# JiawangBian/SC-SfMLearner-Release

Hardware: AMD Instinct MI355X
Metric: train images/sec (+ warp-loss ms/step) KITTI 256x832 RN18 (higher is better)
Workload: dtype f32; 1 GPU; configs[1]: kitti 256x832, batch 12/GPU, 2 refs (seq 3), ResNet18 DispNet + ResNet18 PoseNet, ssim+mask+auto-mask, zeros padding, 1 scale; global_batch=12, parallelism=1 GPU, memory_format=contiguous (NCHW)

## Files before the change

__graft_entry__.py:

```python
import os
import sys

ROOT = os.path.dirname(os.path.abspath(__file__))
PKG = os.path.join(ROOT, "sc-sfmlearner-release_amd")
for p in (ROOT, PKG):
    if p not in sys.path:
        sys.path.insert(0, p)


def build() -> None:
    from scsfm_hip import _lib, build as hip_build
    path = hip_build.build(force=False)
    lib = _lib.CLib(path)
    assert lib._dll.scsfm_abi_version() == _lib.ABI_VERSION
    nets_path = hip_build.build_nets(force=False)
    nets = _lib.CLib(nets_path, _lib.NETS_HEADER, _lib.NETS_ABI_VERSION, "scsfm_nets_")
    eval_path = hip_build.build_eval(force=False)
    ev = _lib.CLib(eval_path, _lib.EVAL_HEADER, _lib.EVAL_ABI_VERSION, "scsfm_eval_")
    odom_path = hip_build.build_odom(force=False)
    od = _lib.CLib(odom_path, _lib.ODOM_HEADER, _lib.ODOM_ABI_VERSION, "scsfm_odom_")
    enc_path = hip_build.build_enc(force=False)
    enc = _lib.CLib(enc_path, _lib.ENC_HEADER, _lib.ENC_ABI_VERSION, "scsfm_enc_")
    stem_path = hip_build.build_stem(force=False)
    stem = _lib.CLib(stem_path, _lib.STEM_HEADER, _lib.STEM_ABI_VERSION, "scsfm_stem_")
    snip_path = hip_build.build_snip(force=False)
    snip = _lib.CLib(snip_path, _lib.SNIP_HEADER, _lib.SNIP_ABI_VERSION, "scsfm_snip_")
    prep_path = hip_build.build_prep(force=False)
    prep = _lib.CLib(prep_path, _lib.PREP_HEADER, _lib.PREP_ABI_VERSION, "scsfm_prep_")
    vis_path = hip_build.build_vis(force=False)
    vis = _lib.CLib(vis_path, _lib.VIS_HEADER, _lib.VIS_ABI_VERSION, "scsfm_vis_")
    dvis_path = hip_build.build_dvis(force=False)
    dvis = _lib.CLib(dvis_path, _lib.DVIS_HEADER, _lib.DVIS_ABI_VERSION, "scsfm_dvis_")
    val_path = hip_build.build_val(force=False)
    val = _lib.CLib(val_path, _lib.VAL_HEADER, _lib.VAL_ABI_VERSION, "scsfm_val_")
    enceval_path = hip_build.build_enceval(force=False)
    enceval = _lib.CLib(enceval_path, _lib.ENCEVAL_HEADER, _lib.ENCEVAL_ABI_VERSION, "scsfm_enceval_")
    decb_path = hip_build.build_decb(force=False)
    decb = _lib.CLib(decb_path, _lib.DECB_HEADER, _lib.DECB_ABI_VERSION, "scsfm_decb_")
    wrw_path = hip_build.build_wrw(force=False)
    wrw = _lib.CLib(wrw_path, _lib.WRW_HEADER, _lib.WRW_ABI_VERSION, "scsfm_wrw_")
    vlog_path = hip_build.build_vlog(force=False)
    vlog = _lib.CLib(vlog_path, _lib.VLOG_HEADER, _lib.VLOG_ABI_VERSION, "scsfm_vlog_")
    import inverse_warp
    import loss_functions
    import models
    from scsfm_hip import decoder, depth_eval, depth_vis, encoder, odometry, prepare, snippets, visualise
    from scsfm_hip import conv_wrw, decoder_bias, encoder_eval, validation, validation_log
    from oracle import scsfm_oracle
    print(f"[vlog:build] {vlog_path}: {len(vlog.decls)} entry points resolved")
    print(f"[wrw:build] {wrw_path}: {len(wrw.decls)} entry points resolved")
    print(f"[decb:build] {decb_path}: {len(decb.decls)} entry points resolved")
    print(f"[enceval:build] {enceval_path}: {len(enceval.decls)} entry points resolved")
    print(f"[val:build] {val_path}: {len(val.decls)} entry points resolved")
    print(f"[build:dvis] {dvis_path}: {len(dvis.decls)} entry points resolved")
    print(f"[build] {path}: {len(lib.decls)} entry points resolved")
    print(f"[build] {nets_path}: {len(nets.decls)} entry points resolved")
    print(f"[build] {eval_path}: {len(ev.decls)} entry points resolved")
    print(f"[build] {odom_path}: {len(od.decls)} entry points resolved")
    print(f"[build] {enc_path}: {len(enc.decls)} entry points resolved")
    print(f"[build] {stem_path}: {len(stem.decls)} entry points resolved")
    print(f"[build] {snip_path}: {len(snip.decls)} entry points resolved")
    print(f"[build:vis] {vis_path}: {len(vis.decls)} entry points resolved")
    print(f"[build:prep] {prep_path}: {len(prep.decls)} entry points resolved")


def smoke() -> None:
    import torch

    import loss_functions as LF
    from oracle import scsfm_oracle as O
    from scsfm_hip import _lib, synth

    assert torch.cuda.is_available(), "smoke() needs a HIP device"
    lib = _lib.get()
    assert lib.path.endswith("libscsfm_hip.so")
    dev = torch.device("cuda:0")
    d = synth.make_batch(2, 128, 416, n_ref=2, seed=0, depth="smooth")

    def leaves(device):
        mv = lambda t: t.to(device).clone().requires_grad_(True)
        return ([mv(t) for t in d["tgt_depth"]], [[mv(t) for t in r] for r in d["ref_depths"]],
# ... 86 lines not shown
    assert _lib.get_enceval().path.endswith("libscsfm_enceval.so")
    bn_e = nn.BatchNorm2d(4).to(dev)
    with torch.no_grad():
        bn_e.running_mean.copy_(torch.tensor([0.5, -1.0, 0.0, 2.0]))
        bn_e.running_var.copy_(torch.tensor([0.25, 1.0, 4.0, 0.5]))
        bn_e.weight.copy_(torch.tensor([1.0, -0.5, 2.0, 0.0]))
        bn_e.bias.copy_(torch.tensor([0.0, 0.1, -0.2, 0.3]))
    bn_e.eval()
    with torch.no_grad():
        f0_e, pooled_e = EE.bn_act(xs, bn_e, pool=True)
        want_e = F.relu(bn_e(xs))
        assert torch.equal(f0_e, EE.bn_act(xs, bn_e)) and torch.equal(pooled_e, F.max_pool2d(f0_e, 3, 2, 1))
        assert torch.equal(pooled_e, EE.max_pool(f0_e))
    err_e = float((f0_e - want_e).abs().max())
    print(f"[smoke] enceval: eval-mode BatchNorm / ReLU / max-pool, max |fused - ATen| {err_e:.2e}")
    assert err_e <= 1e-5
    from scsfm_hip import decoder_bias as DB
    assert _lib.get_decb().path.endswith("libscsfm_decb.so")
    conv_b = nn.Conv2d(4, 3, 3).to(dev)
    xb = torch.randn(2, 4, 9, 11, device=dev)
    want_b = F.pad(F.elu(conv_b(xb)), (1, 1, 1, 1), mode="reflect")
    want_h = 10 * torch.sigmoid(conv_b(xb)) + 0.01
    (want_b.sum() + want_h.sum()).backward()
    want_gb = conv_b.bias.grad.clone()
    conv_b.bias.grad = None
    raw = F.conv2d(xb, conv_b.weight, None)
    got_b, got_h = DB.elu_pad(raw, conv_b.bias), DB.disp_head(raw, conv_b.bias, 10, 0.01)
    (got_b.sum() + got_h.sum()).backward()
    err_b = float((conv_b.bias.grad - want_gb).abs().max() / want_gb.abs().max())
    print(f"[smoke] decb: bias folded into elu_pad and disp_head, relative bias-gradient difference {err_b:.2e}")
    assert torch.equal(got_b, want_b) and float((got_h - want_h).abs().max()) <= 1e-6 and err_b <= 1e-5
    _smoke_wrw(dev)
    _smoke_vlog(dev)
    print("[smoke] ok")


def _smoke_wrw(dev) -> None:
    import torch
    import torch.nn.functional as F

    from scsfm_hip import _lib
    from scsfm_hip import conv_wrw as CW
    assert _lib.get_wrw().path.endswith("libscsfm_wrw.so")
    xw = torch.randn(2, 16, 7, 69, device=dev, requires_grad=True)
    ww = torch.randn(16, 16, 3, 3, device=dev, requires_grad=True)
    gy = torch.randn(2, 16, 5, 67, device=dev)
    gx_w, gw_w = torch.autograd.grad(CW.conv3x3_valid(xw, ww), (xw, ww), gy)
    gx_m, gw_m = torch.autograd.grad(F.conv2d(xw, ww), (xw, ww), gy)
    gw_64 = torch.autograd.grad(F.conv2d(xw.double(), ww.double()), ww, gy.double())[0]
    s_64 = torch.autograd.grad(F.conv2d(xw.double().abs(), ww.double()), ww, gy.double().abs())[0]
    err_w, err_m = float((gw_w - gw_64).abs().max()), float((gw_m - gw_64).abs().max())
    print(f"[smoke] wrw: weight gradient of a 16 -> 16 convolution, max |hip - fp64| {err_w:.2e} (MIOpen's {err_m:.2e})")
    assert float((gx_w - gx_m).abs().max()) <= 1e-5 * float(gx_m.abs().max())
    assert err_w <= 2 * err_m + 8 * 2.0 ** -24 * float(s_64.max())
    assert torch.equal(gw_w, CW.weight_grad(xw.detach(), gy))


def _smoke_vlog(dev) -> None:
    import numpy as np
    import torch

    from scsfm_hip import _lib
    from scsfm_hip import validation_log as VL
    assert _lib.get_vlog().path.endswith("libscsfm_vlog.so")
    ramp = torch.linspace(0.05, 12.0, 35).reshape(1, 5, 7)
    r = ramp.numpy()
    for cmap, max_value in (("magma", None), ("rainbow", 10)):
        floats, rgba = VL.map_pictures(ramp.to(dev), cmap, max_value)
        table = VL.colour_table_f32(cmap)
        d = r.max() if max_value is None else np.float32(max_value)
        xa = (r / d).astype(np.float32) * np.float32(len(table))
        want = table[np.clip(xa.astype(np.int64), 0, len(table) - 1)]
        assert floats.shape == (1, 4, 5, 7) and np.array_equal(floats.cpu().numpy(), want.transpose(0, 3, 1, 2)), cmap
        assert rgba.shape == (1, 5, 7, 4) and np.array_equal(rgba.cpu().numpy(), VL.to_bytes(want)), cmap
        assert torch.equal(VL.tensor2array(ramp[0].to(dev), max_value, cmap), floats[0])
    print("[smoke] vlog: magma and rainbow pictures of a ramp equal the table lookup, as floats and as bytes")


if __name__ == "__main__":
    build()
    if "--smoke" in sys.argv:
        smoke()
```

sc-sfmlearner-release_amd/models/DispResNet.py:

```python
from __future__ import absolute_import, division, print_function

import numpy as np
import torch
import torch.nn as nn
import torch.nn.functional as F

from .resnet_encoder import ResnetEncoder


class Conv3x3(nn.Module):
    def __init__(self, in_channels, out_channels, use_refl=True):
        super().__init__()
        self.pad = nn.ReflectionPad2d(1) if use_refl else nn.ZeroPad2d(1)
        self.conv = nn.Conv2d(int(in_channels), int(out_channels), 3)

    def forward(self, x):
        return self.conv(self.pad(x))


class ConvBlock(nn.Module):
    def __init__(self, in_channels, out_channels):
        super().__init__()
        self.conv = Conv3x3(in_channels, out_channels)
        self.nonlin = nn.ELU(inplace=True)
# ... 54 lines not shown
            x = self.decoder[self._up[(i, 0)]](x)
            x = F.interpolate(x, scale_factor=2, mode="nearest")
            if self.use_skips and i > 0:
                x = torch.cat([x, feats[i - 1]], 1)
            x = self.decoder[self._up[(i, 1)]](x)
            if i in self._head:
                outputs.append(self.alpha * self.sigmoid(self.decoder[self._head[i]](x)) + self.beta)
        return outputs[::-1]

    def forward_fused(self, feats):
        from scsfm_hip import conv_wrw as CW, decoder as D

        def conv(k, x):
            m = self._conv(k)
            if CW.applies(x, m):
                y = CW.conv3x3_valid(x, m.weight)
                return y if m.bias is None else y + m.bias.view(1, -1, 1, 1)
            return m(x)

        outputs = []
        x = D.pad(feats[-1])
        for i in range(4, -1, -1):
            a = conv(self._up[(i, 0)], x)
            x = D.up_cat_pad(a, feats[i - 1] if self.use_skips and i > 0 else None)
            b = conv(self._up[(i, 1)], x)
            if i == 0 and i not in self._head:
                break
            x = D.elu_pad(b)
            if i in self._head:
                outputs.append(self.alpha * self.sigmoid(conv(self._head[i], x)) + self.beta)
        return outputs[::-1]

    def forward_fused_bias(self, feats):
        from scsfm_hip import conv_wrw as CW, decoder as D, decoder_bias as DB

        def conv(k, x):
            m = self._conv(k)
            if CW.applies(x, m):
                return CW.conv3x3_valid(x, m.weight), m.bias
            return F.conv2d(x, m.weight, None, m.stride, m.padding, m.dilation, m.groups), m.bias

        outputs = []
        x = D.pad(feats[-1])
        for i in range(4, -1, -1):
            a, bias = conv(self._up[(i, 0)], x)
            x = DB.up_cat_pad(a, bias, feats[i - 1] if self.use_skips and i > 0 else None)
            if i == 0 and i not in self._head:
                self._conv(self._up[(i, 1)])(x)
                break
            b, bias = conv(self._up[(i, 1)], x)
            x = DB.elu_pad(b, bias)
            if i in self._head:
                h, bias = conv(self._head[i], x)
                outputs.append(DB.disp_head(h, bias, self.alpha, self.beta))
        return outputs[::-1]


class DispResNet(nn.Module):
    def __init__(self, num_layers=18, pretrained=True):
        super().__init__()
        self.encoder = ResnetEncoder(num_layers=num_layers, pretrained=pretrained, num_input_images=1)
        self.decoder = DepthDecoder(self.encoder.num_ch_enc)

    def init_weights(self):
        pass

    def forward(self, x):
        outputs = self.decoder(self.encoder(x))
        return outputs if self.training else outputs[0]
```

sc-sfmlearner-release_amd/scsfm_hip/_lib.py:

```python
from __future__ import annotations

import ctypes
import os
import re
import threading

import torch

HERE = os.path.dirname(os.path.abspath(__file__))
HEADER = os.path.join(os.path.dirname(os.path.dirname(HERE)), "include", "scsfm_hip.h")
LIB_PATH = os.environ.get("SCSFM_HIP_LIB") or os.path.join(HERE, "libscsfm_hip.so")

ABI_VERSION = 9

_CTYPES = {"int": ctypes.c_int, "unsigned": ctypes.c_uint, "size_t": ctypes.c_size_t, "double": ctypes.c_double,
           "float": ctypes.c_float}
_DECL = re.compile(r"^(int|size_t)\s+(scsfm_\w+)\s*\(([^)]*)\)\s*;", re.M | re.S)


def parse_header(path=HEADER):
    text = open(path).read()
    text = re.sub(r"/\*.*?\*/", "", text, flags=re.S)
    out = {}
    for ret, name, args in _DECL.findall(text):
# ... 420 lines not shown
                lib = CLib(WRW_LIB_PATH, WRW_HEADER, WRW_ABI_VERSION, "scsfm_wrw_")
                if lib.source_id() != _build.wrw_source_id():
                    raise ScsfmError(f"{WRW_LIB_PATH}: its source id {lib.source_id()} is not the tree's "
                                     f"{_build.wrw_source_id()}")
                _wrw = lib
    return _wrw


VLOG_HEADER = os.path.join(os.path.dirname(os.path.dirname(HERE)), "include", "scsfm_vlog.h")
VLOG_LIB_PATH = os.path.join(HERE, "libscsfm_vlog.so")
VLOG_ABI_VERSION = 1
_vlog = None


def get_vlog() -> CLib:
    global _vlog
    if _vlog is None:
        with _lock:
            if _vlog is None:
                from . import build as _build
                if _build.vlog_is_stale():
                    have = _build.binary_source_id(VLOG_LIB_PATH)
                    try:
                        _build.build_vlog()
                    except Exception as e:
                        raise ScsfmError(f"{VLOG_LIB_PATH} is stale or missing ({have}) and cannot be built here: {e}") \
                            from e
                lib = CLib(VLOG_LIB_PATH, VLOG_HEADER, VLOG_ABI_VERSION, "scsfm_vlog_")
                if lib.source_id() != _build.vlog_source_id():
                    raise ScsfmError(f"{VLOG_LIB_PATH}: its source id {lib.source_id()} is not the tree's "
                                     f"{_build.vlog_source_id()}")
                _vlog = lib
    return _vlog
```

sc-sfmlearner-release_amd/scsfm_hip/build.py:

```python
from __future__ import annotations

import contextlib
import fcntl
import glob
import hashlib
import os
import shutil
import subprocess
import sys
import tempfile

HERE = os.path.dirname(os.path.abspath(__file__))
CSRC = os.path.join(os.path.dirname(HERE), "csrc")
LIB = os.path.join(HERE, "libscsfm_hip.so")
LOCK = LIB + ".lock"
LOG = LIB + ".buildlog"
INCLUDE = os.path.join(os.path.dirname(os.path.dirname(HERE)), "include")
NETS_CSRC = os.path.join(os.path.dirname(HERE), "csrc_nets")
NETS_LIB = os.path.join(HERE, "libscsfm_nets.so")
EVAL_CSRC = os.path.join(os.path.dirname(HERE), "csrc_eval")
EVAL_LIB = os.path.join(HERE, "libscsfm_eval.so")
ODOM_CSRC = os.path.join(os.path.dirname(HERE), "csrc_odom")
ODOM_LIB = os.path.join(HERE, "libscsfm_odom.so")
ENC_CSRC = os.path.join(os.path.dirname(HERE), "csrc_enc")
ENC_LIB = os.path.join(HERE, "libscsfm_enc.so")
STEM_CSRC = os.path.join(os.path.dirname(HERE), "csrc_stem")
STEM_LIB = os.path.join(HERE, "libscsfm_stem.so")
SNIP_CSRC = os.path.join(os.path.dirname(HERE), "csrc_snip")
SNIP_LIB = os.path.join(HERE, "libscsfm_snip.so")
PREP_CSRC = os.path.join(os.path.dirname(HERE), "csrc_prep")
PREP_LIB = os.path.join(HERE, "libscsfm_prep.so")
VIS_CSRC = os.path.join(os.path.dirname(HERE), "csrc_vis")
VIS_LIB = os.path.join(HERE, "libscsfm_vis.so")
DVIS_CSRC = os.path.join(os.path.dirname(HERE), "csrc_dvis")
DVIS_LIB = os.path.join(HERE, "libscsfm_dvis.so")
VAL_CSRC = os.path.join(os.path.dirname(HERE), "csrc_val")
VAL_LIB = os.path.join(HERE, "libscsfm_val.so")
ENCEVAL_CSRC = os.path.join(os.path.dirname(HERE), "csrc_enceval")
ENCEVAL_LIB = os.path.join(HERE, "libscsfm_enceval.so")
DECB_CSRC = os.path.join(os.path.dirname(HERE), "csrc_decb")
DECB_LIB = os.path.join(HERE, "libscsfm_decb.so")
WRW_CSRC = os.path.join(os.path.dirname(HERE), "csrc_wrw")
WRW_LIB = os.path.join(HERE, "libscsfm_wrw.so")
VLOG_CSRC = os.path.join(os.path.dirname(HERE), "csrc_vlog")
VLOG_LIB = os.path.join(HERE, "libscsfm_vlog.so")
ARCH = "gfx950"
FLAGS = ["-O3", "-std=c++17", "-fPIC", "-shared", f"--offload-arch={ARCH}", "-munsafe-fp-atomics",
         "-fno-gpu-rdc", "-Wall", "-Wno-unused-function",
         "-fno-slp-vectorize"]
ID_MARKER = b"scsfm-source-id:"


def sources():
    return sorted(glob.glob(os.path.join(CSRC, "*.hip")))


def deps():
    return sources() + sorted(glob.glob(os.path.join(CSRC, "*.h"))) + \
        [os.path.join(INCLUDE, "scsfm_hip.h")]


def nets_sources():
    return sorted(glob.glob(os.path.join(NETS_CSRC, "*.hip")))


def nets_deps():
    return nets_sources() + sorted(glob.glob(os.path.join(NETS_CSRC, "*.h"))) + [os.path.join(INCLUDE, "scsfm_nets.h")]


def eval_sources():
    return sorted(glob.glob(os.path.join(EVAL_CSRC, "*.hip")))


def eval_deps():
    return eval_sources() + sorted(glob.glob(os.path.join(EVAL_CSRC, "*.h"))) + [os.path.join(INCLUDE, "scsfm_eval.h")]


def odom_sources():
# ... 61 lines not shown


def enceval_sources():
    return sorted(glob.glob(os.path.join(ENCEVAL_CSRC, "*.hip")))


def enceval_deps():
    return enceval_sources() + sorted(glob.glob(os.path.join(ENCEVAL_CSRC, "*.h"))) + \
        [os.path.join(INCLUDE, "scsfm_enceval.h")]


def decb_sources():
    return sorted(glob.glob(os.path.join(DECB_CSRC, "*.hip")))


def decb_deps():
    return decb_sources() + sorted(glob.glob(os.path.join(DECB_CSRC, "*.h"))) + [os.path.join(INCLUDE, "scsfm_decb.h")]


def wrw_sources():
    return sorted(glob.glob(os.path.join(WRW_CSRC, "*.hip")))


def wrw_deps():
    return wrw_sources() + sorted(glob.glob(os.path.join(WRW_CSRC, "*.h"))) + [os.path.join(INCLUDE, "scsfm_wrw.h")]


def vlog_sources():
    return sorted(glob.glob(os.path.join(VLOG_CSRC, "*.hip")))


def vlog_deps():
    return vlog_sources() + sorted(glob.glob(os.path.join(VLOG_CSRC, "*.h"))) + [os.path.join(INCLUDE, "scsfm_vlog.h")]


def _hash(files, extra=()):
    h = hashlib.sha256()
    for path in files:
        h.update(os.path.basename(path).encode())
        h.update(open(path, "rb").read())
    h.update(" ".join(FLAGS).encode())
    if extra:
        h.update(b"\0extra:" + " ".join(extra).encode())
    return h.hexdigest()[:16]


def source_id(extra=()):
    files = deps()
    if any("SCSFM_WITH_MARCH" in e or "variants" in e for e in extra):
        vsrc = os.path.join(os.path.dirname(os.path.dirname(HERE)), "variants", "src")
        files = files + sorted(p for p in glob.glob(os.path.join(vsrc, "*")) if os.path.isfile(p))
    return _hash(files, extra)


def nets_source_id():
    return _hash(nets_deps())


def eval_source_id():
    return _hash(eval_deps())


def odom_source_id():
    return _hash(odom_deps())


# ... 9 lines not shown
    return _hash(snip_deps())


def prep_source_id():
    return _hash(prep_deps())


def vis_source_id():
    return _hash(vis_deps())


def dvis_source_id():
    return _hash(dvis_deps())


def val_source_id():
    return _hash(val_deps())


def enceval_source_id():
    return _hash(enceval_deps())


def decb_source_id():
    return _hash(decb_deps())


def wrw_source_id():
    return _hash(wrw_deps())


def vlog_source_id():
    return _hash(vlog_deps())


def binary_source_id(path=LIB):
    try:
        blob = open(path, "rb").read()
    except OSError:
        return None
    i = blob.find(ID_MARKER)
    if i < 0:
        return None
    j = i + len(ID_MARKER)
    return blob[j:j + 16].decode("ascii", "replace")


def is_stale():
    return binary_source_id(LIB) != source_id()


def nets_is_stale():
    return binary_source_id(NETS_LIB) != nets_source_id()


def eval_is_stale():
    return binary_source_id(EVAL_LIB) != eval_source_id()


def odom_is_stale():
    return binary_source_id(ODOM_LIB) != odom_source_id()


def enc_is_stale():
    return binary_source_id(ENC_LIB) != enc_source_id()

# ... 6 lines not shown
    return binary_source_id(SNIP_LIB) != snip_source_id()


def prep_is_stale():
    return binary_source_id(PREP_LIB) != prep_source_id()


def vis_is_stale():
    return binary_source_id(VIS_LIB) != vis_source_id()


def dvis_is_stale():
    return binary_source_id(DVIS_LIB) != dvis_source_id()


def val_is_stale():
    return binary_source_id(VAL_LIB) != val_source_id()


def enceval_is_stale():
    return binary_source_id(ENCEVAL_LIB) != enceval_source_id()


def decb_is_stale():
    return binary_source_id(DECB_LIB) != decb_source_id()


def wrw_is_stale():
    return binary_source_id(WRW_LIB) != wrw_source_id()


def vlog_is_stale():
    return binary_source_id(VLOG_LIB) != vlog_source_id()


@contextlib.contextmanager
def _build_lock(lock=None):
    fd = os.open(lock or LOCK, os.O_CREAT | os.O_RDWR, 0o644)
    try:
        fcntl.flock(fd, fcntl.LOCK_EX)
        yield
    finally:
        try:
            fcntl.flock(fd, fcntl.LOCK_UN)
        finally:
            os.close(fd)


def build(force=False, verbose=True, extra=()):
    extra = tuple(extra)
    return _build(LIB, source_id(extra), sources(), extra, force, verbose)


def build_nets(force=False, verbose=True):
    return _build(NETS_LIB, nets_source_id(), nets_sources(), ("-I", INCLUDE), force, verbose)


def build_eval(force=False, verbose=True):
    return _build(EVAL_LIB, eval_source_id(), eval_sources(), ("-I", INCLUDE), force, verbose)


def build_odom(force=False, verbose=True):
    return _build(ODOM_LIB, odom_source_id(), odom_sources(), ("-I", INCLUDE), force, verbose)


def build_enc(force=False, verbose=True):
# ... 8 lines not shown
    return _build(SNIP_LIB, snip_source_id(), snip_sources(), ("-I", INCLUDE), force, verbose)


def build_prep(force=False, verbose=True):
    return _build(PREP_LIB, prep_source_id(), prep_sources(), ("-I", INCLUDE), force, verbose)


def build_vis(force=False, verbose=True):
    return _build(VIS_LIB, vis_source_id(), vis_sources(), ("-I", INCLUDE), force, verbose)


def build_dvis(force=False, verbose=True):
    return _build(DVIS_LIB, dvis_source_id(), dvis_sources(), ("-I", INCLUDE), force, verbose)


def build_val(force=False, verbose=True):
    return _build(VAL_LIB, val_source_id(), val_sources(), ("-I", INCLUDE), force, verbose)


def build_enceval(force=False, verbose=True):
    return _build(ENCEVAL_LIB, enceval_source_id(), enceval_sources(), ("-I", INCLUDE), force, verbose)


def build_decb(force=False, verbose=True):
    return _build(DECB_LIB, decb_source_id(), decb_sources(), ("-I", INCLUDE), force, verbose)


def build_wrw(force=False, verbose=True):
    return _build(WRW_LIB, wrw_source_id(), wrw_sources(), ("-I", INCLUDE), force, verbose)


def build_vlog(force=False, verbose=True):
    return _build(VLOG_LIB, vlog_source_id(), vlog_sources(), ("-I", INCLUDE), force, verbose)


def _build(lib, want, srcs, extra, force, verbose):
    if not force and binary_source_id(lib) == want:
        return lib
    with _build_lock(lib + ".lock"):
        if not force and binary_source_id(lib) == want:
            return lib
        hipcc = shutil.which("hipcc") or "/opt/rocm/bin/hipcc"
        name = os.path.basename(lib)
        if not os.path.exists(hipcc):
            raise RuntimeError(f"hipcc not found: {name} cannot be built on this machine")
        fd, tmp = tempfile.mkstemp(prefix=name[:-len(".so")] + ".", suffix=f".{os.getpid()}.tmp", dir=HERE)
        os.close(fd)
        try:
            cmd = [hipcc, *FLAGS, f'-DSCSFM_SOURCE_ID="{want}"', *extra, "-o", tmp, *srcs]
            if verbose:
                print("[scsfm_hip.build]", " ".join(cmd), flush=True)
            subprocess.run(cmd, check=True)
            os.chmod(tmp, 0o755)
            os.replace(tmp, lib)
            with open(lib + ".buildlog", "a") as f:
                f.write(f"{want} {os.getpid()}\n")
        finally:
            if os.path.exists(tmp):
                os.unlink(tmp)
    return lib


if __name__ == "__main__":
    build(force="--force" in sys.argv)
    build_nets(force="--force" in sys.argv)
    build_eval(force="--force" in sys.argv)
    build_odom(force="--force" in sys.argv)
    build_enc(force="--force" in sys.argv)
    build_stem(force="--force" in sys.argv)
    build_snip(force="--force" in sys.argv)
    build_prep(force="--force" in sys.argv)
    build_vis(force="--force" in sys.argv)
    build_dvis(force="--force" in sys.argv)
    build_val(force="--force" in sys.argv)
    build_enceval(force="--force" in sys.argv)
    build_decb(force="--force" in sys.argv)
    build_wrw(force="--force" in sys.argv)
    build_vlog(force="--force" in sys.argv)
    print(LIB)
    print(NETS_LIB)
    print(EVAL_LIB)
    print(ODOM_LIB)
    print(ENC_LIB)
    print(STEM_LIB)
    print(SNIP_LIB)
    print(PREP_LIB)
    print(VIS_LIB)
    print(DVIS_LIB)
    print(VAL_LIB)
    print(ENCEVAL_LIB)
    print(DECB_LIB)
    print(WRW_LIB)
    print(VLOG_LIB)
```

sc-sfmlearner-release_amd/scsfm_hip/config.py:

```python
from __future__ import annotations

_hint = (1.0, 0.5)
_hint_dev = {}


def set_weight_hint(w_photo, w_geom):
    global _hint
    if w_photo is None:
        _hint = None
        return
    import numpy as np
    _hint = (float(np.float32(w_photo)), float(np.float32(w_geom)))
    for t in _hint_dev.values():
        t.copy_(t.new_tensor(_hint))


def weight_hint():
    return _hint


def hint_tensor(device):
    if _hint is None:
        return None
    import torch
# ... 42 lines not shown
    _errors_torch = bool(on)


_decoder_bias = None


def decoder_bias_folded():
    global _decoder_bias
    if _decoder_bias is None:
        import os
        _decoder_bias = os.environ.get("SCSFM_DECODER_BIAS", "1") != "0"
    return _decoder_bias


def set_decoder_bias_folded(on):
    global _decoder_bias
    _decoder_bias = None if on is None else bool(on)


_decoder_wrw = None


def decoder_wrw():
    global _decoder_wrw
    if _decoder_wrw is None:
        import os
        _decoder_wrw = os.environ.get("SCSFM_DECODER_WRW", "1") != "0"
    return _decoder_wrw


def set_decoder_wrw(on):
    global _decoder_wrw
    _decoder_wrw = None if on is None else bool(on)
```

sc-sfmlearner-release_amd/scsfm_hip/conv_wrw.py:

```python
from __future__ import annotations

import torch
import torch.nn.functional as F

from . import _lib, config
from .capi import _stream

COUT = (1, 16, 32)
CIN = (16, 32, 64, 96)
ROUTED = {(64, 32), (96, 32), (32, 16), (16, 16), (64, 1), (32, 1), (16, 1)}


def covers(cin, cout):
    return int(cin) in CIN and int(cout) in COUT


def applies(x, m):
    w = m.weight
    return (config.decoder_wrw() and x.is_cuda and x.dtype == torch.float32 and x.dim() == 4 and x.is_contiguous()
            and w.is_cuda and w.dtype == torch.float32 and w.is_contiguous() and tuple(w.shape[2:]) == (3, 3)
            and tuple(m.stride) == (1, 1) and tuple(m.padding) == (0, 0) and tuple(m.dilation) == (1, 1)
            and m.groups == 1 and m.padding_mode == "zeros" and x.shape[1] == w.shape[1]
            and (int(w.shape[1]), int(w.shape[0])) in ROUTED and x.shape[2] >= 3 and x.shape[3] >= 3)


def weight_grad(x, gy):
    B, Cin, Hp, Wp = x.shape
    Cout, H, W = gy.shape[1], Hp - 2, Wp - 2
    if not (x.is_cuda and gy.is_cuda and x.dtype == gy.dtype == torch.float32 and x.is_contiguous()
            and gy.is_contiguous() and tuple(gy.shape) == (B, Cout, H, W)):
        raise ValueError(f"scsfm_hip.conv_wrw: CUDA fp32 contiguous x[B, Cin, H + 2, W + 2] and gy[B, Cout, H, W] only "
                         f"(got {x.device} {x.dtype} {tuple(x.shape)} and {gy.device} {gy.dtype} {tuple(gy.shape)})")
    lib = _lib.get_wrw()
    n = lib.size("scsfm_wrw_conv3x3_ws_bytes", B, Cin, Cout, H, W)
    if n == 0:
        raise ValueError(f"scsfm_hip.conv_wrw: no kernel for {Cin} -> {Cout} channels at {B} x {H} x {W}")
    ws = torch.empty(n // 4, dtype=torch.float32, device=x.device)
    dw = torch.empty((Cout, Cin, 3, 3), dtype=torch.float32, device=x.device)
    lib.call("scsfm_wrw_conv3x3_f32", B, Cin, Cout, H, W, x.data_ptr(), gy.data_ptr(), dw.data_ptr(), ws.data_ptr(), n,
             _stream(x))
    return dw


class _Conv3x3Valid(torch.autograd.Function):
    @staticmethod
    def forward(ctx, x, weight):
        ctx.save_for_backward(x, weight)
        return F.conv2d(x, weight)

    @staticmethod
    def backward(ctx, gy):
        x, weight = ctx.saved_tensors
        gy = gy.contiguous()
        gx = gw = None
        if ctx.needs_input_grad[0]:
            gx = torch.ops.aten.convolution_backward(gy, x, weight, None, [1, 1], [0, 0], [1, 1], False, [0, 0], 1,
                                                     [True, False, False])[0]
        if ctx.needs_input_grad[1]:
            gw = weight_grad(x, gy)
        return gx, gw


def conv3x3_valid(x_padded, weight):
    return _Conv3x3Valid.apply(x_padded, weight)
```

Baseline: 149.4 images/s.

## Fuse disparity head tail backward and add MFMA conv3x3 data-gradient kernel

Adds a HIP library with two kernels. The first runs the whole backward of the final decoder stage (sigmoid-scaled disparity head, its 16->1 conv data gradient with reflect-pad folding, and ELU backward) in one kernel, with fp64 bias-gradient sums. The second is an MFMA-based 16/32<-16 channel 3x3 conv data-gradient kernel that replaces MIOpen's backward-data call for routed decoder convs. Both aim to cut kernel launches, intermediate memory traffic and MIOpen overhead in the decoder backward pass, at the cost of more custom code and border-handling complexity.

```diff
diff --git a/__graft_entry__.py b/__graft_entry__.py
--- a/__graft_entry__.py
+++ b/__graft_entry__.py
@@ -41,12 +41,15 @@
     wrw = _lib.CLib(wrw_path, _lib.WRW_HEADER, _lib.WRW_ABI_VERSION, "scsfm_wrw_")
     vlog_path = hip_build.build_vlog(force=False)
     vlog = _lib.CLib(vlog_path, _lib.VLOG_HEADER, _lib.VLOG_ABI_VERSION, "scsfm_vlog_")
+    dgrad_path = hip_build.build_dgrad(force=False)
+    dgrad = _lib.CLib(dgrad_path, _lib.DGRAD_HEADER, _lib.DGRAD_ABI_VERSION, "scsfm_dgrad_")
     import inverse_warp
     import loss_functions
     import models
     from scsfm_hip import decoder, depth_eval, depth_vis, encoder, odometry, prepare, snippets, visualise
-    from scsfm_hip import conv_wrw, decoder_bias, encoder_eval, validation, validation_log
+    from scsfm_hip import conv_wrw, decoder_bias, decoder_dgrad, encoder_eval, validation, validation_log
     from oracle import scsfm_oracle
+    print(f"[dgrad:build] {dgrad_path}: {len(dgrad.decls)} entry points resolved")
     print(f"[vlog:build] {vlog_path}: {len(vlog.decls)} entry points resolved")
     print(f"[wrw:build] {wrw_path}: {len(wrw.decls)} entry points resolved")
     print(f"[decb:build] {decb_path}: {len(decb.decls)} entry points resolved")
@@ -199,6 +202,7 @@
     assert torch.equal(got_b, want_b) and float((got_h - want_h).abs().max()) <= 1e-6 and err_b <= 1e-5
     _smoke_wrw(dev)
     _smoke_vlog(dev)
+    _smoke_dgrad(dev)
     print("[smoke] ok")
 
 
@@ -244,6 +248,42 @@
     print("[smoke] vlog: magma and rainbow pictures of a ramp equal the table lookup, as floats and as bytes")
 
 
+def _smoke_dgrad(dev) -> None:
+    import torch
+    import torch.nn.functional as F
+
+    from scsfm_hip import _lib
+    from scsfm_hip import decoder_bias as DB, decoder_dgrad as DG
+    assert _lib.get_dgrad().path.endswith("libscsfm_dgrad.so")
+    g = torch.Generator().manual_seed(3)
+    b, bias = torch.randn(2, 16, 5, 67, generator=g), torch.randn(16, generator=g)
+    wh, bh = torch.randn(1, 16, 3, 3, generator=g) / 12, torch.randn(1, generator=g)
+    gy = torch.randn(2, 1, 5, 67, generator=g)
+    leaves = lambda dtype: [t.to(dev, dtype).requires_grad_(True) for t in (b, bias, wh, bh)]
+
+    def chain(b, bias, wh, bh):
+        q = F.pad(F.elu(b + bias.view(1, -1, 1, 1)), (1, 1, 1, 1), mode="reflect")
+        return 10 * torch.sigmoid(F.conv2d(q, wh, bh)) + 0.01
+    x32, x64 = leaves(torch.float32), leaves(torch.float64)
+    out = DG.head_tail(*x32, 10, 0.01)
+    got = torch.autograd.grad(out, x32, gy.to(dev))
+    want = torch.autograd.grad(chain(*x64), x64, gy.to(dev).double())
+    with torch.no_grad():
+        parts = DB.disp_head(F.conv2d(DB.elu_pad(x32[0], x32[1]), x32[2]), x32[3], 10, 0.01)
+    assert torch.equal(out, parts)
+    err = max(float((a.double() - c).abs().max() / c.abs().max()) for a, c in zip(got, want))
+    print(f"[smoke] dgrad: the tail's backward in one kernel, largest relative gradient difference to fp64 {err:.2e}")
+    assert err <= 1e-5
+    from scsfm_hip import conv_wrw as CW
+    gyc, wc = torch.randn(2, 16, 5, 67, generator=g).to(dev), torch.randn(16, 16, 3, 3, generator=g).to(dev)
+    xc = torch.zeros(2, 16, 7, 69, device=dev)
+    want_c = torch.ops.aten.convolution_backward(gyc, xc, wc, None, [1, 1], [0, 0], [1, 1], False, [0, 0], 1,
+                                                 [True, False, False])[0]
+    err_c = float((CW.data_grad(gyc, wc) - want_c).abs().max() / want_c.abs().max())
+    print(f"[smoke] dgrad: data gradient of a 16 -> 16 convolution, relative difference to MIOpen's {err_c:.2e}")
+    assert err_c <= 1e-5
+
+
 if __name__ == "__main__":
     build()
     if "--smoke" in sys.argv:
diff --git a/include/scsfm_dgrad.h b/include/scsfm_dgrad.h
--- /dev/null
+++ b/include/scsfm_dgrad.h
@@ -0,0 +1,30 @@
+#ifndef SCSFM_DGRAD_H_
+#define SCSFM_DGRAD_H_
+
+#include <stddef.h>
+
+#ifndef SCSFM_ERR_ARG
+#define SCSFM_ERR_ARG (-1)
+#endif
+
+#ifdef __cplusplus
+extern "C" {
+#endif
+
+int scsfm_dgrad_abi_version(void);
+int scsfm_dgrad_source_id(char* buf, size_t n);
+int scsfm_dgrad_head_tail_covers(int C);
+size_t scsfm_dgrad_head_tail_ws_bytes(int B, int C, int H, int W);
+int scsfm_dgrad_head_tail_bwd_f32(int B, int C, int H, int W, float alpha, const float* q, const float* y,
+                                  const float* g_out, const float* w, float* g, float* g_b, void* ws, size_t ws_bytes,
+                                  float* g_bias_b, float* g_bias_head, void* stream);
+
+int scsfm_dgrad_conv3x3_covers(int Cin, int Cout);
+int scsfm_dgrad_conv3x3_f32(int B, int Cin, int Cout, int H, int W, const float* dy, const float* w, float* dx,
+                            void* stream);
+
+#ifdef __cplusplus
+}
+#endif
+
+#endif
diff --git a/sc-sfmlearner-release_amd/csrc_dgrad/scsfm_conv_dgrad.hip b/sc-sfmlearner-release_amd/csrc_dgrad/scsfm_conv_dgrad.hip
--- /dev/null
+++ b/sc-sfmlearner-release_amd/csrc_dgrad/scsfm_conv_dgrad.hip
@@ -0,0 +1,125 @@
+#include <hip/hip_runtime.h>
+
+#include "scsfm_dgrad.h"
+
+#ifndef SCSFM_WRW_F32X4
+typedef float f32x4 __attribute__((ext_vector_type(4)));
+#endif
+
+namespace scsfm_dgrad_conv {
+
+constexpr int kCout = 16;
+constexpr int kWave = 64;
+constexpr int kWaves = 4;
+constexpr int kThreads = kWave * kWaves;
+constexpr int kTP = 8, kTQ = 64;
+constexpr int kLH = kTP + 2, kLW = kTQ + 2;
+constexpr int kPlane = 672;
+constexpr int kSteps = 36;
+constexpr int kBatch = 14;
+
+template <int NB>
+__global__ __launch_bounds__(kThreads) void conv3x3_dgrad_kernel(int H, int W, int tiles_q, int tiles_p,
+                                                                  const float* __restrict__ dy,
+                                                                  const float* __restrict__ w, float* __restrict__ dx) {
+  __shared__ float tile[kCout * kPlane];
+  constexpr int Cin = 16 * NB;
+  const int tid = threadIdx.x, lane = tid & (kWave - 1), wv = tid >> 6;
+  const int col = lane & 15, quad = lane >> 4;
+  int t = blockIdx.x;
+  const int tq = t % tiles_q;
+  t /= tiles_q;
+  const int tp = t % tiles_p, n = t / tiles_p;
+  const int p0 = tp * kTP, q0 = tq * kTQ;
+  const int Hp = H + 2, Wp = W + 2;
+
+  float a[NB][kSteps];
+#pragma unroll
+  for (int m = 0; m < NB; ++m)
+#pragma unroll
+    for (int rs = 0; rs < 9; ++rs)
+#pragma unroll
+      for (int g = 0; g < 4; ++g) a[m][rs * 4 + g] = w[((4 * g + quad) * Cin + 16 * m + col) * 9 + rs];
+
+  constexpr int kElems = kCout * kLH * kLW;
+  for (int e0 = tid; e0 < kElems; e0 += kBatch * kThreads) {
+    float v[kBatch];
+    int at[kBatch];
+#pragma unroll
+    for (int u = 0; u < kBatch; ++u) {
+      const int e = e0 + u * kThreads;
+      const int co = e / (kLH * kLW), rem = e - co * (kLH * kLW);
+      const int lr = rem / kLW, lc = rem - lr * kLW;
+      const int gi = p0 - 2 + lr, gj = q0 - 2 + lc;
+      at[u] = e < kElems ? co * kPlane + rem : -1;
+      v[u] = 0.f;
+      if (e < kElems && gi >= 0 && gi < H && gj >= 0 && gj < W) v[u] = dy[((n * kCout + co) * H + gi) * W + gj];
+    }
+#pragma unroll
+    for (int u = 0; u < kBatch; ++u)
+      if (at[u] >= 0) tile[at[u]] = v[u];
+  }
+  __syncthreads();
+
+#pragma unroll 1
+  for (int k = 0; k < kTP / kWaves; ++k) {
+    const int lp = wv + k * kWaves, p = p0 + lp;
+#pragma unroll 1
+    for (int cb = 0; cb < kTQ / 16; ++cb) {
+      f32x4 acc[NB];
+#pragma unroll
+      for (int m = 0; m < NB; ++m) acc[m] = f32x4{0.f, 0.f, 0.f, 0.f};
+      const float* base = tile + quad * kPlane + (lp + 2) * kLW + cb * 16 + col + 2;
+#pragma unroll
+      for (int r = 0; r < 3; ++r)
+#pragma unroll
+        for (int s = 0; s < 3; ++s)
+#pragma unroll
+          for (int g = 0; g < 4; ++g) {
+            const float b = base[4 * g * kPlane - r * kLW - s];
+#pragma unroll
+            for (int m = 0; m < NB; ++m)
+              acc[m] = __builtin_amdgcn_mfma_f32_16x16x4f32(a[m][(r * 3 + s) * 4 + g], b, acc[m], 0, 0, 0);
+          }
+      const int q = q0 + cb * 16 + col;
+      if (p < Hp && q < Wp) {
+#pragma unroll
+        for (int m = 0; m < NB; ++m)
+#pragma unroll
+          for (int i = 0; i < 4; ++i) dx[((n * Cin + 16 * m + 4 * quad + i) * Hp + p) * Wp + q] = acc[m][i];
+      }
+    }
+  }
+}
+
+inline int ceil_div(int a, int b) { return (a + b - 1) / b; }
+
+inline long long workgroups(int B, int Cin, int Cout, int H, int W) {
+  if (B <= 0 || Cout != kCout || (Cin != 16 && Cin != 32) || H < 1 || W < 1) return 0;
+  if ((long long)B * (Cin > Cout ? Cin : Cout) * (H + 2ll) * (W + 2ll) >= (1ll << 31)) return 0;
+  return (long long)B * ceil_div(H + 2, kTP) * ceil_div(W + 2, kTQ);
+}
+
+}
+
+using namespace scsfm_dgrad_conv;
+
+extern "C" {
+
+int scsfm_dgrad_conv3x3_covers(int Cin, int Cout) { return Cout == kCout && (Cin == 16 || Cin == 32) ? 1 : 0; }
+
+int scsfm_dgrad_conv3x3_f32(int B, int Cin, int Cout, int H, int W, const float* dy, const float* w, float* dx,
+                            void* stream) {
+  const long long nwg = workgroups(B, Cin, Cout, H, W);
+  if (nwg == 0 || !dy || !w || !dx) return SCSFM_ERR_ARG;
+  (void)hipGetLastError();
+  const int tiles_q = ceil_div(W + 2, kTQ), tiles_p = ceil_div(H + 2, kTP);
+  const dim3 grid((unsigned)nwg), block(kThreads);
+  if (Cin == 16)
+    hipLaunchKernelGGL(conv3x3_dgrad_kernel<1>, grid, block, 0, (hipStream_t)stream, H, W, tiles_q, tiles_p, dy, w, dx);
+  else
+    hipLaunchKernelGGL(conv3x3_dgrad_kernel<2>, grid, block, 0, (hipStream_t)stream, H, W, tiles_q, tiles_p, dy, w, dx);
+  return (int)hipGetLastError();
+}
+
+}
diff --git a/sc-sfmlearner-release_amd/csrc_dgrad/scsfm_decoder_dgrad.hip b/sc-sfmlearner-release_amd/csrc_dgrad/scsfm_decoder_dgrad.hip
--- /dev/null
+++ b/sc-sfmlearner-release_amd/csrc_dgrad/scsfm_decoder_dgrad.hip
@@ -0,0 +1,218 @@
+#include <hip/hip_runtime.h>
+
+#include <stdint.h>
+
+#include "scsfm_dgrad.h"
+
+#pragma clang fp contract(off)
+
+namespace scsfm_dgrad {
+
+constexpr int kC = 16;
+constexpr int kWave = 64;
+constexpr int kWaves = 4;
+constexpr int kThreads = kWave * kWaves;
+constexpr int kTW = 64, kTH = 8;
+constexpr int kLW = kTW + 2, kLH = kTH + 2;
+constexpr int kSums = kC + 1;
+
+__device__ inline float elu_grad(float g, float r) { return r <= 0.f ? g * (r + 1.f) : g; }
+
+__device__ inline double wave_sum(double v) {
+#pragma unroll
+  for (int d = kWave / 2; d > 0; d >>= 1) v += __shfl_down(v, d);
+  return v;
+}
+
+template <bool SUM>
+__global__ __launch_bounds__(kThreads) void head_tail_bwd_kernel(int H, int W, int tiles_x, int tiles_y, float alpha,
+                                                                  const float* __restrict__ q,
+                                                                  const float* __restrict__ y,
+                                                                  const float* __restrict__ g_out,
+                                                                  const float* __restrict__ w, float* __restrict__ g,
+                                                                  float* __restrict__ g_b, double* __restrict__ ws) {
+  __shared__ float tile[kLH * kLW];
+  __shared__ double red[kWaves][kSums];
+  const int tid = threadIdx.x, lane = tid & (kWave - 1), wv = tid >> 6;
+  int t = blockIdx.x;
+  const int tx = t % tiles_x;
+  t /= tiles_x;
+  const int ty = t % tiles_y, b = t / tiles_y;
+  const int i0 = ty * kTH, j0 = tx * kTW;
+
+  for (int e = tid; e < kLH * kLW; e += kThreads) {
+    const int li = e / kLW, lj = e - li * kLW;
+    const int gi = i0 + li - 1, gj = j0 + lj - 1;
+    float v = 0.f;
+    if (gi >= 0 && gi < H && gj >= 0 && gj < W) {
+      const int idx = (b * H + gi) * W + gj;
+      v = g_out[idx];
+      if (y) {
+        const float s = y[idx];
+        v = ((v * alpha) * (1.f - s)) * s;
+      }
+      if (li >= 1 && li <= kTH && lj >= 1 && lj <= kTW) g[idx] = v;
+    }
+    tile[e] = v;
+  }
+  __syncthreads();
+
+  const int Hp = H + 2, Wp = W + 2;
+  const int j = j0 + lane;
+  double sum[kSums];
+#pragma unroll
+  for (int c = 0; c < kSums; ++c) sum[c] = 0.0;
+
+  auto gat = [&](int gi, int gj) -> float {
+    return gi >= 0 && gi < H && gj >= 0 && gj < W ? tile[(gi - i0 + 1) * kLW + (gj - j0 + 1)] : 0.f;
+  };
+  auto gq = [&](const float* wc, int p, int qq) -> float {
+    float a = 0.f;
+#pragma unroll
+    for (int r = 0; r < 3; ++r)
+#pragma unroll
+      for (int s = 0; s < 3; ++s) a += wc[r * 3 + s] * gat(p - r, qq - s);
+    return a;
+  };
+
+#pragma unroll
+  for (int k = 0; k < kTH / kWaves; ++k) {
+    const int li = wv + k * kWaves, i = i0 + li;
+    if (i < H && j < W) {
+      const float* tp = tile + (li + 1) * kLW + lane + 1;
+      float G[3][3];
+#pragma unroll
+      for (int a = 0; a < 3; ++a)
+#pragma unroll
+        for (int c = 0; c < 3; ++c) G[a][c] = tp[(a - 1) * kLW + (c - 1)];
+      const bool border = i == 1 || i == H - 2 || j == 1 || j == W - 2;
+      const float* qp = q + ((b * kC) * Hp + i + 1) * Wp + j + 1;
+      float* dst = g_b + ((b * kC) * H + i) * W + j;
+      float r[kC];
+#pragma unroll
+      for (int c = 0; c < kC; ++c) r[c] = qp[c * Hp * Wp];
+#pragma unroll
+      for (int c = 0; c < kC; ++c) {
+        const float* wc = w + c * 9;
+        float in = 0.f;
+#pragma unroll
+        for (int rr = 0; rr < 3; ++rr)
+#pragma unroll
+          for (int s = 0; s < 3; ++s) in += wc[rr * 3 + s] * G[2 - rr][2 - s];
+        float acc = in;
+        if (border) {
+          acc = 0.f;
+          acc += in;
+          if (j == 1) acc += gq(wc, i + 1, 0);
+          if (j == W - 2) acc += gq(wc, i + 1, W + 1);
+          auto row = [&](int p) {
+            acc += gq(wc, p, j + 1);
+            if (j == 1) acc += gq(wc, p, 0);
+            if (j == W - 2) acc += gq(wc, p, W + 1);
+          };
+          if (i == 1) row(0);
+          if (i == H - 2) row(H + 1);
+        }
+        const float f = elu_grad(acc, r[c]);
+        dst[c * H * W] = f;
+        if (SUM) sum[c] += (double)f;
+      }
+      if (SUM) sum[kC] += (double)G[1][1];
+    }
+  }
+
+  if (SUM) {
+#pragma unroll
+    for (int c = 0; c < kSums; ++c) {
+      const double v = wave_sum(sum[c]);
+      if (lane == 0) red[wv][c] = v;
+    }
+    __syncthreads();
+    if (tid < kSums) {
+      double v = red[0][tid];
+#pragma unroll
+      for (int k = 1; k < kWaves; ++k) v += red[k][tid];
+      ws[tid * gridDim.x + blockIdx.x] = v;
+    }
+  }
+}
+
+static __global__ __launch_bounds__(kThreads) void sums_kernel(int n, const double* __restrict__ ws,
+                                                                float* __restrict__ g_bias_b,
+                                                                float* __restrict__ g_bias_head) {
+  __shared__ double red[kWaves];
+  const int c = blockIdx.x;
+  float* dst = c < kC ? (g_bias_b ? g_bias_b + c : nullptr) : g_bias_head;
+  if (!dst) return;
+  double s = 0.0;
+  for (int k = threadIdx.x; k < n; k += kThreads) s += ws[c * n + k];
+  s = wave_sum(s);
+  if ((threadIdx.x & (kWave - 1)) == 0) red[threadIdx.x >> 6] = s;
+  __syncthreads();
+  if (threadIdx.x == 0) {
+    double v = red[0];
+#pragma unroll
+    for (int k = 1; k < kWaves; ++k) v += red[k];
+    *dst = (float)v;
+  }
+}
+
+inline int ceil_div(int a, int b) { return (a + b - 1) / b; }
+
+inline long long workgroups(int B, int C, int H, int W) {
+  if (B <= 0 || C != kC || H < 2 || W < 2) return 0;
+  if ((long long)B * C * (H + 2ll) * (W + 2ll) >= (1ll << 31)) return 0;
+  return (long long)B * ceil_div(H, kTH) * ceil_div(W, kTW);
+}
+
+}
+
+using namespace scsfm_dgrad;
+
+extern "C" {
+
+int scsfm_dgrad_abi_version(void) { return 1; }
+
+#ifndef SCSFM_SOURCE_ID
+#define SCSFM_SOURCE_ID "unknown"
+#endif
+static const char g_source_tag[] __attribute__((used)) = "scsfm-source-id:" SCSFM_SOURCE_ID;
+int scsfm_dgrad_source_id(char* buf, size_t n) {
+  const volatile char* id = g_source_tag + 16;
+  if (!buf || n == 0) return -1;
+  size_t i = 0;
+  for (; i + 1 < n && id[i]; ++i) buf[i] = id[i];
+  buf[i] = 0;
+  return 0;
+}
+
+int scsfm_dgrad_head_tail_covers(int C) { return C == kC ? 1 : 0; }
+
+size_t scsfm_dgrad_head_tail_ws_bytes(int B, int C, int H, int W) {
+  return sizeof(double) * kSums * (size_t)workgroups(B, C, H, W);
+}
+
+int scsfm_dgrad_head_tail_bwd_f32(int B, int C, int H, int W, float alpha, const float* q, const float* y,
+                                  const float* g_out, const float* w, float* g, float* g_b, void* ws, size_t ws_bytes,
+                                  float* g_bias_b, float* g_bias_head, void* stream) {
+  const long long nwg = workgroups(B, C, H, W);
+  const bool sum = g_bias_b || g_bias_head;
+  if (nwg == 0 || !q || !g_out || !w || !g || !g_b) return SCSFM_ERR_ARG;
+  if (sum && (!ws || ((uintptr_t)ws & 7) || ws_bytes < sizeof(double) * kSums * (size_t)nwg)) return SCSFM_ERR_ARG;
+  (void)hipGetLastError();
+  const int tiles_x = ceil_div(W, kTW), tiles_y = ceil_div(H, kTH);
+  const dim3 grid((unsigned)nwg), block(kThreads);
+  if (!sum) {
+    hipLaunchKernelGGL(head_tail_bwd_kernel<false>, grid, block, 0, (hipStream_t)stream, H, W, tiles_x, tiles_y, alpha,
+                       q, y, g_out, w, g, g_b, (double*)nullptr);
+    return (int)hipGetLastError();
+  }
+  hipLaunchKernelGGL(head_tail_bwd_kernel<true>, grid, block, 0, (hipStream_t)stream, H, W, tiles_x, tiles_y, alpha, q,
+                     y, g_out, w, g, g_b, (double*)ws);
+  if (const int rc = (int)hipGetLastError()) return rc;
+  hipLaunchKernelGGL(sums_kernel, dim3(kSums), block, 0, (hipStream_t)stream, (int)nwg, (const double*)ws, g_bias_b,
+                     g_bias_head);
+  return (int)hipGetLastError();
+}
+
+}
diff --git a/sc-sfmlearner-release_amd/models/DispResNet.py b/sc-sfmlearner-release_amd/models/DispResNet.py
--- a/sc-sfmlearner-release_amd/models/DispResNet.py
+++ b/sc-sfmlearner-release_amd/models/DispResNet.py
@@ -110,12 +110,14 @@
         return outputs[::-1]
 
     def forward_fused_bias(self, feats):
-        from scsfm_hip import conv_wrw as CW, decoder as D, decoder_bias as DB
+        from scsfm_hip import conv_wrw as CW, decoder as D, decoder_bias as DB, decoder_dgrad as DG
 
         def conv(k, x):
             m = self._conv(k)
             if CW.applies(x, m):
                 return CW.conv3x3_valid(x, m.weight), m.bias
+            if CW.applies_without_wrw(x, m):
+                return CW.conv3x3_valid(x, m.weight, wrw=False), m.bias
             return F.conv2d(x, m.weight, None, m.stride, m.padding, m.dilation, m.groups), m.bias
 
         outputs = []
@@ -127,6 +129,10 @@
                 self._conv(self._up[(i, 1)])(x)
                 break
             b, bias = conv(self._up[(i, 1)], x)
+            if i == 0 and DG.applies(b, bias, self._conv(self._head[0])):
+                head = self._conv(self._head[0])
+                outputs.append(DG.head_tail(b, bias, head.weight, head.bias, self.alpha, self.beta))
+                break
             x = DB.elu_pad(b, bias)
             if i in self._head:
                 h, bias = conv(self._head[i], x)
diff --git a/sc-sfmlearner-release_amd/scsfm_hip/_lib.py b/sc-sfmlearner-release_amd/scsfm_hip/_lib.py
--- a/sc-sfmlearner-release_amd/scsfm_hip/_lib.py
+++ b/sc-sfmlearner-release_amd/scsfm_hip/_lib.py
@@ -476,3 +476,30 @@
                                      f"{_build.vlog_source_id()}")
                 _vlog = lib
     return _vlog
+
+
+DGRAD_HEADER = os.path.join(os.path.dirname(os.path.dirname(HERE)), "include", "scsfm_dgrad.h")
+DGRAD_LIB_PATH = os.path.join(HERE, "libscsfm_dgrad.so")
+DGRAD_ABI_VERSION = 1
+_dgrad = None
+
+
+def get_dgrad() -> CLib:
+    global _dgrad
+    if _dgrad is None:
+        with _lock:
+            if _dgrad is None:
+                from . import build as _build
+                if _build.dgrad_is_stale():
+                    have = _build.binary_source_id(DGRAD_LIB_PATH)
+                    try:
+                        _build.build_dgrad()
+                    except Exception as e:
+                        raise ScsfmError(f"{DGRAD_LIB_PATH} is stale or missing ({have}) and cannot be built here: {e}") \
+                            from e
+                lib = CLib(DGRAD_LIB_PATH, DGRAD_HEADER, DGRAD_ABI_VERSION, "scsfm_dgrad_")
+                if lib.source_id() != _build.dgrad_source_id():
+                    raise ScsfmError(f"{DGRAD_LIB_PATH}: its source id {lib.source_id()} is not the tree's "
+                                     f"{_build.dgrad_source_id()}")
+                _dgrad = lib
+    return _dgrad
diff --git a/sc-sfmlearner-release_amd/scsfm_hip/build.py b/sc-sfmlearner-release_amd/scsfm_hip/build.py
--- a/sc-sfmlearner-release_amd/scsfm_hip/build.py
+++ b/sc-sfmlearner-release_amd/scsfm_hip/build.py
@@ -44,6 +44,8 @@
 WRW_LIB = os.path.join(HERE, "libscsfm_wrw.so")
 VLOG_CSRC = os.path.join(os.path.dirname(HERE), "csrc_vlog")
 VLOG_LIB = os.path.join(HERE, "libscsfm_vlog.so")
+DGRAD_CSRC = os.path.join(os.path.dirname(HERE), "csrc_dgrad")
+DGRAD_LIB = os.path.join(HERE, "libscsfm_dgrad.so")
 ARCH = "gfx950"
 FLAGS = ["-O3", "-std=c++17", "-fPIC", "-shared", f"--offload-arch={ARCH}", "-munsafe-fp-atomics",
          "-fno-gpu-rdc", "-Wall", "-Wno-unused-function",
@@ -171,6 +173,15 @@
 
 def vlog_deps():
     return vlog_sources() + sorted(glob.glob(os.path.join(VLOG_CSRC, "*.h"))) + [os.path.join(INCLUDE, "scsfm_vlog.h")]
+
+
+def dgrad_sources():
+    return sorted(glob.glob(os.path.join(DGRAD_CSRC, "*.hip")))
+
+
+def dgrad_deps():
+    return dgrad_sources() + sorted(glob.glob(os.path.join(DGRAD_CSRC, "*.h"))) + \
+        [os.path.join(INCLUDE, "scsfm_dgrad.h")]
 
 
 def _hash(files, extra=()):
@@ -246,6 +257,10 @@
 
 def vlog_source_id():
     return _hash(vlog_deps())
+
+
+def dgrad_source_id():
+    return _hash(dgrad_deps())
 
 
 def binary_source_id(path=LIB):
@@ -318,6 +333,10 @@
 
 def vlog_is_stale():
     return binary_source_id(VLOG_LIB) != vlog_source_id()
+
+
+def dgrad_is_stale():
+    return binary_source_id(DGRAD_LIB) != dgrad_source_id()
 
 
 @contextlib.contextmanager
@@ -392,6 +411,10 @@
 
 def build_vlog(force=False, verbose=True):
     return _build(VLOG_LIB, vlog_source_id(), vlog_sources(), ("-I", INCLUDE), force, verbose)
+
+
+def build_dgrad(force=False, verbose=True):
+    return _build(DGRAD_LIB, dgrad_source_id(), dgrad_sources(), ("-I", INCLUDE), force, verbose)
 
 
 def _build(lib, want, srcs, extra, force, verbose):
@@ -437,6 +460,7 @@
     build_decb(force="--force" in sys.argv)
     build_wrw(force="--force" in sys.argv)
     build_vlog(force="--force" in sys.argv)
+    build_dgrad(force="--force" in sys.argv)
     print(LIB)
     print(NETS_LIB)
     print(EVAL_LIB)
@@ -452,3 +476,4 @@
     print(DECB_LIB)
     print(WRW_LIB)
     print(VLOG_LIB)
+    print(DGRAD_LIB)
diff --git a/sc-sfmlearner-release_amd/scsfm_hip/config.py b/sc-sfmlearner-release_amd/scsfm_hip/config.py
--- a/sc-sfmlearner-release_amd/scsfm_hip/config.py
+++ b/sc-sfmlearner-release_amd/scsfm_hip/config.py
@@ -98,3 +98,19 @@
 def set_decoder_wrw(on):
     global _decoder_wrw
     _decoder_wrw = None if on is None else bool(on)
+
+
+_decoder_dgrad = None
+
+
+def decoder_dgrad():
+    global _decoder_dgrad
+    if _decoder_dgrad is None:
+        import os
+        _decoder_dgrad = os.environ.get("SCSFM_DECODER_DGRAD", "1") != "0"
+    return _decoder_dgrad
+
+
+def set_decoder_dgrad(on):
+    global _decoder_dgrad
+    _decoder_dgrad = None if on is None else bool(on)
diff --git a/sc-sfmlearner-release_amd/scsfm_hip/conv_wrw.py b/sc-sfmlearner-release_amd/scsfm_hip/conv_wrw.py
--- a/sc-sfmlearner-release_amd/scsfm_hip/conv_wrw.py
+++ b/sc-sfmlearner-release_amd/scsfm_hip/conv_wrw.py
@@ -9,19 +9,36 @@
 COUT = (1, 16, 32)
 CIN = (16, 32, 64, 96)
 ROUTED = {(64, 32), (96, 32), (32, 16), (16, 16), (64, 1), (32, 1), (16, 1)}
+DGRAD_COUT = (16,)
+DGRAD_CIN = (16, 32)
+ROUTED_DGRAD = {(16, 16), (32, 16)}
 
 
 def covers(cin, cout):
     return int(cin) in CIN and int(cout) in COUT
 
 
-def applies(x, m):
+def dgrad_covers(cin, cout):
+    return int(cin) in DGRAD_CIN and int(cout) in DGRAD_COUT
+
+
+def _plain3x3(x, m):
     w = m.weight
-    return (config.decoder_wrw() and x.is_cuda and x.dtype == torch.float32 and x.dim() == 4 and x.is_contiguous()
+    return (x.is_cuda and x.dtype == torch.float32 and x.dim() == 4 and x.is_contiguous()
             and w.is_cuda and w.dtype == torch.float32 and w.is_contiguous() and tuple(w.shape[2:]) == (3, 3)
             and tuple(m.stride) == (1, 1) and tuple(m.padding) == (0, 0) and tuple(m.dilation) == (1, 1)
             and m.groups == 1 and m.padding_mode == "zeros" and x.shape[1] == w.shape[1]
-            and (int(w.shape[1]), int(w.shape[0])) in ROUTED and x.shape[2] >= 3 and x.shape[3] >= 3)
+            and x.shape[2] >= 3 and x.shape[3] >= 3)
+
+
+def applies(x, m):
+    w = m.weight
+    return bool(config.decoder_wrw() and _plain3x3(x, m) and (int(w.shape[1]), int(w.shape[0])) in ROUTED)
+
+
+def applies_without_wrw(x, m):
+    w = m.weight
+    return bool(config.decoder_dgrad() and _plain3x3(x, m) and (int(w.shape[1]), int(w.shape[0])) in ROUTED_DGRAD)
 
 
 def weight_grad(x, gy):
@@ -42,10 +59,30 @@
     return dw
 
 
+def data_grad_routed(gy, weight):
+    return (config.decoder_dgrad() and gy.is_cuda and gy.dtype == torch.float32 and gy.is_contiguous()
+            and weight.is_cuda and weight.dtype == torch.float32 and weight.is_contiguous()
+            and (int(weight.shape[1]), int(weight.shape[0])) in ROUTED_DGRAD)
+
+
+def data_grad(gy, weight):
+    B, Cout, H, W = gy.shape
+    Cin = weight.shape[1]
+    if not (gy.is_cuda and weight.is_cuda and gy.dtype == weight.dtype == torch.float32 and gy.is_contiguous()
+            and weight.is_contiguous() and tuple(weight.shape) == (Cout, Cin, 3, 3) and dgrad_covers(Cin, Cout)):
+        raise ValueError(f"scsfm_hip.conv_wrw: CUDA fp32 contiguous gy[B, 16, H, W] and weight[16, 16 | 32, 3, 3] only "
+                         f"(got {gy.device} {gy.dtype} {tuple(gy.shape)} and {weight.dtype} {tuple(weight.shape)})")
+    dx = torch.empty((B, Cin, H + 2, W + 2), dtype=torch.float32, device=gy.device)
+    _lib.get_dgrad().call("scsfm_dgrad_conv3x3_f32", B, Cin, Cout, H, W, gy.data_ptr(), weight.data_ptr(),
+                          dx.data_ptr(), _stream(gy))
+    return dx
+
+
 class _Conv3x3Valid(torch.autograd.Function):
     @staticmethod
-    def forward(ctx, x, weight):
+    def forward(ctx, x, weight, wrw=True):
         ctx.save_for_backward(x, weight)
+        ctx.wrw = wrw
         return F.conv2d(x, weight)
 
     @staticmethod
@@ -53,13 +90,18 @@
         x, weight = ctx.saved_tensors
         gy = gy.contiguous()
         gx = gw = None
+
+        def miopen(k):
+            mask = [k == 0, k == 1, False]
+            return torch.ops.aten.convolution_backward(gy, x, weight, None, [1, 1], [0, 0], [1, 1], False, [0, 0], 1,
+                                                       mask)[k]
+
         if ctx.needs_input_grad[0]:
-            gx = torch.ops.aten.convolution_backward(gy, x, weight, None, [1, 1], [0, 0], [1, 1], False, [0, 0], 1,
-                                                     [True, False, False])[0]
+            gx = data_grad(gy, weight) if data_grad_routed(gy, weight) else miopen(0)
         if ctx.needs_input_grad[1]:
-            gw = weight_grad(x, gy)
-        return gx, gw
+            gw = weight_grad(x, gy) if ctx.wrw else miopen(1)
+        return gx, gw, None
 
 
-def conv3x3_valid(x_padded, weight):
-    return _Conv3x3Valid.apply(x_padded, weight)
+def conv3x3_valid(x_padded, weight, wrw=True):
+    return _Conv3x3Valid.apply(x_padded, weight, bool(wrw))
diff --git a/sc-sfmlearner-release_amd/scsfm_hip/decoder_dgrad.py b/sc-sfmlearner-release_amd/scsfm_hip/decoder_dgrad.py
--- /dev/null
+++ b/sc-sfmlearner-release_amd/scsfm_hip/decoder_dgrad.py
@@ -0,0 +1,104 @@
+from __future__ import annotations
+
+import torch
+import torch.nn.functional as F
+
+from . import _lib, config, conv_wrw
+from .capi import _stream
+from .decoder import _check, _padded
+from .decoder_bias import _check_bias, _ptr
+
+CHANNELS = (16,)
+
+
+def covers(C):
+    return int(C) in CHANNELS
+
+
+def _plain(t, dim):
+    return t is not None and t.is_cuda and t.dtype == torch.float32 and t.dim() == dim and t.is_contiguous()
+
+
+def applies(b, bias_b, head):
+    w = head.weight
+    return (config.decoder_dgrad() and _plain(b, 4) and _plain(bias_b, 1) and _plain(w, 4) and _plain(head.bias, 1)
+            and covers(b.shape[1]) and tuple(w.shape) == (1, b.shape[1], 3, 3) and bias_b.shape[0] == b.shape[1]
+            and tuple(head.stride) == (1, 1) and tuple(head.padding) == (0, 0) and tuple(head.dilation) == (1, 1)
+            and head.groups == 1 and head.padding_mode == "zeros" and b.shape[2] >= 2 and b.shape[3] >= 2)
+
+
+def tail_bwd(q, y, g_out, weight, alpha, want_bias_b=True, want_bias_head=True):
+    B, C, Hp, Wp = q.shape
+    H, W = Hp - 2, Wp - 2
+    _check(q, y, g_out, weight)
+    if not (tuple(g_out.shape) == (B, 1, H, W) and (y is None or y.shape == g_out.shape)
+            and tuple(weight.shape) == (1, C, 3, 3)):
+        raise ValueError(f"scsfm_hip.decoder_dgrad: q {tuple(q.shape)}, g_out {tuple(g_out.shape)} and weight "
+                         f"{tuple(weight.shape)} do not belong together")
+    lib = _lib.get_dgrad()
+    n = lib.size("scsfm_dgrad_head_tail_ws_bytes", B, C, H, W)
+    if n == 0:
+        raise ValueError(f"scsfm_hip.decoder_dgrad: no kernel for {C} channels at {B} x {H} x {W}")
+    g = torch.empty_like(g_out)
+    g_b = torch.empty((B, C, H, W), dtype=q.dtype, device=q.device)
+    ws = torch.empty(n // 8, dtype=torch.float64, device=q.device) if want_bias_b or want_bias_head else None
+    g_bias_b = torch.empty(C, dtype=q.dtype, device=q.device) if want_bias_b else None
+    g_bias_head = torch.empty(1, dtype=q.dtype, device=q.device) if want_bias_head else None
+    lib.call("scsfm_dgrad_head_tail_bwd_f32", B, C, H, W, float(alpha), q.data_ptr(), _ptr(y), g_out.data_ptr(),
+             weight.data_ptr(), g.data_ptr(), g_b.data_ptr(), _ptr(ws), n if ws is not None else 0, _ptr(g_bias_b),
+             _ptr(g_bias_head), _stream(q))
+    return g, g_b, g_bias_b, g_bias_head
+
+
+def _head_weight_grad(q, g, weight):
+    if config.decoder_wrw() and (int(q.shape[1]), 1) in conv_wrw.ROUTED:
+        return conv_wrw.weight_grad(q, g)
+    return torch.ops.aten.convolution_backward(g, q, weight, None, [1, 1], [0, 0], [1, 1], False, [0, 0], 1,
+                                               [False, True, False])[1]
+
+
+class _HeadTail(torch.autograd.Function):
+    @staticmethod
+    def forward(ctx, b, bias_b, head_weight, head_bias, alpha, beta):
+        _check(b, head_weight)
+        B, C, H, W = b.shape
+        _check_bias(bias_b, C)
+        _check_bias(head_bias, 1)
+        decb = _lib.get_decb()
+        q = _padded(b, C, H, W)
+        decb.call("scsfm_decb_bias_elu_pad_fwd_f32", B, C, H, W, b.data_ptr(), bias_b.data_ptr(), q.data_ptr(),
+                  _stream(b))
+        h = F.conv2d(q, head_weight)
+        y, out = torch.empty_like(h), torch.empty_like(h)
+        decb.call("scsfm_decb_disp_head_fwd_f32", B, 1, H, W, h.data_ptr(), head_bias.data_ptr(), float(alpha),
+                  float(beta), y.data_ptr(), out.data_ptr(), _stream(b))
+        ctx.save_for_backward(q, y, head_weight)
+        ctx.alpha = float(alpha)
+        return out
+
+    @staticmethod
+    def backward(ctx, g_out):
+        g_out = g_out.contiguous()
+        q, y, head_weight = ctx.saved_tensors
+        need_b, need_bias_b, need_w, need_bias_h = ctx.needs_input_grad[:4]
+        g = g_b = g_bias_b = g_bias_h = g_w = None
+        if need_b or need_bias_b:
+            g, g_b, g_bias_b, g_bias_h = tail_bwd(q, y, g_out, head_weight, ctx.alpha, need_bias_b, need_bias_h)
+        elif need_w or need_bias_h:
+            B, _, H, W = y.shape
+            decb = _lib.get_decb()
+            g = torch.empty_like(y)
+            ws = None
+            if need_bias_h:
+                ws = torch.empty(decb.size("scsfm_decb_ws_bytes", B, 1, 1, H * W) // 8, dtype=torch.float64,
+                                 device=y.device)
+                g_bias_h = torch.empty(1, dtype=y.dtype, device=y.device)
+            decb.call("scsfm_decb_disp_head_bwd_f32", B, 1, H, W, ctx.alpha, g_out.data_ptr(), y.data_ptr(),
+                      g.data_ptr(), _ptr(ws), _ptr(g_bias_h), _stream(y))
+        if need_w:
+            g_w = _head_weight_grad(q, g, head_weight)
+        return (g_b if need_b else None), g_bias_b, g_w, g_bias_h, None, None
+
+
+def head_tail(b, bias_b, head_weight, head_bias, alpha, beta):
+    return _HeadTail.apply(b, bias_b, head_weight, head_bias, alpha, beta)
```

After: 151.0 images/s (median of 6 runs). 1.01x the previous value.
